# liron88/HM-16.2

Hardware: AMD Instinct MI355X
Metric: CTUs/sec (enc) at 4K main10; bit-exact CU partition vs HM (higher is better)
Workload: dtype int32+f64

## Files before the change

### hm-16.2_amd/csrc/hm355_core.h

```cpp
#pragma once
#include <stddef.h>
#include "hm355_types.h"

#ifdef HM355_HOSTSIM
#include <string.h>
#include <math.h>
#include <stdlib.h>
#define HM_DEV static
#define HM_FINL static inline
#define HM_FINL_M inline
#define HM_LAMBDA_INL
#define HM_NOINLINE __attribute__((noinline))
#define HM_CONST static const
#define HM_ASSUME_LDS(p) ((void)0)
#define HM_ASSUME_GLB(p) ((void)0)
#define HM_NT 1
static inline int hm_lane() { return 0; }
#define HM_SYNC() ((void)0)
static inline uint32_t hm_wave_sum(uint32_t v) { return v; }
static inline int hm_wave_sum_i(int v) { return v; }
static inline int hm_wave_max_i(int v) { return v; }
#define HM_UNI(x) (x)
#define HM_UCALL(x) (x)
#define hm_uni_ptr(p) (p)
// ... 217 lines not shown
struct TZ {
  const Pel *org; int orgStride, w, h;
  const Pel *ref; int refStride;
  uint32_t bestSad; int bestX, bestY, bestDist, bestRound, pointNr;
  int16_t l, r, t, b;
  int16_t subShift, pad_;
  int16_t lx[16], ly[16]; uint16_t lpd[16];
  int16_t wx0, wy0, ww, wh;
};
struct IrqFrame {
  TU t; int8_t phase, child, checkFull, checkSplit, zero; uint8_t bestTS[3];
  uint32_t absSum[3], bestCBF[3], singleBits, singleDist, subBits, subDist; double singleCost, subCost;
};

#define HM_TSTRIDE 33
#define HM_RQ_LDS 256
struct RqLds {
  int32_t lvl[HM_RQ_LDS];
  uint16_t pos[HM_RQ_LDS];
  uint16_t dec[HM_RQ_LDS];
  int16_t cur[HM_RQ_LDS];
  uint8_t ctxSig[HM_RQ_LDS];
  uint8_t code[HM_RQ_LDS];
  uint8_t cgCtxSet[64];
  uint8_t cgFlag[64];
};
struct RefLds {
  Pel refTop[2][132], refLeft[2][132];
  Pel refMain[200], refSide[200];
  Pel line[272];
};
#define HM_SLOT(d, ci) ((d) * CI_NUM + (ci) - ((d) == 4 ? 2 : 0))
#define HM_NUM_SLOTS (4 * CI_NUM + 3)
struct Team;
#if defined(HM355_PROFILE) && !defined(HM355_HOSTSIM)
#define HM_CTU_WAVES 11
#else
#define HM_CTU_WAVES 12
#endif
struct LdsTables {
  int8_t tmat[32 * HM_TSTRIDE];
  int8_t dst4[16];
  int32_t ebits[128];
};
#if defined(HM355_HOSTSIM)
static LdsTables g_lt;
#else
__shared__ LdsTables g_lt;
#endif
#define HM_LT() (&g_lt)
struct Shared {
  Cabac cur;
  int32_t bufA[32 * HM_TSTRIDE];
  union {
    int32_t bufB[32 * HM_TSTRIDE];
    RqLds rq;
    RefLds ref;
  } u;
  TuWalk walkOuter, walkInner;
  CuFrame cuf[4];
  double outCost; uint32_t outBits, outDist; double outRdCost;
  int32_t mpmZ;
  int32_t s8Winner, s8Reuse;
  InterMeta *im;
  uint32_t mcost; MvD mvPredictor; int32_t costScale;
  union {
// ... 1713 lines not shown
    }
    if (n == 4) {
      cabac_copy(&e->cur, &e->ws->slot[HM_SLOT(cuDepth, CI_CURR_BEST)]);
      { HM_PROF_BEGIN(e, PR_S4L); simt4_luma_pu(e, t, numModesForFullRD); HM_PROF_END(e, PR_S4L); }
      overallDistY += e->outDistY;
      if (pu != numPU - 1)
        par_copy_blk(e->fb.rec[0] + (e->ctuY * 64 + t.y) * ps + e->ctuX * 64 + t.x, ps, ws->reco + t.y * 64 + t.x, 64, n);
      continue;
    }
    int bestPUMode = 0; uint32_t bestPUDistY = 0; double bestPUCost = HM_MAX_DOUBLE;
    int firstPass = 0;
    if (n == 8 || n == 16) {
      cabac_copy(&e->cur, &e->ws->slot[HM_SLOT(cuDepth, CI_CURR_BEST)]);
      if (n == 8) { HM_PROF_BEGIN(e, PR_S8L); bestPUMode = HM_UCALL(simt8_luma_first_pass(e, t, numModesForFullRD)); HM_PROF_END(e, PR_S8L); }
      else { HM_PROF_BEGIN(e, PR_S16L); bestPUMode = HM_UCALL(simt16_luma_first_pass(e, t, numModesForFullRD)); HM_PROF_END(e, PR_S16L); }
      firstPass = numModesForFullRD;
      e->s8Reuse = 1;
    }
    for (int pass = firstPass; pass <= numModesForFullRD; pass++) {
      const int last = (pass == numModesForFullRD);
      const int orgMode = last ? bestPUMode : rdModeList[pass];
      par_set8(m->dirL + z, orgMode, puParts);
      cabac_copy(&e->cur, &e->ws->slot[HM_SLOT(cuDepth, CI_CURR_BEST)]);
      e->outCost = bestPUCost;
      if (last && n == 32 && numModesForFullRD > 0) { e->s8Reuse = 2; e->outDistY = bestPUDistY; e->outRdCost = bestPUCost; }
      recur_intra_coding_qt(e, t, !last);
      const uint32_t puDistY = e->outDistY; const double puCost = e->outRdCost;
      if (puCost < bestPUCost) {
        bestPUMode = orgMode; bestPUDistY = puDistY; bestPUCost = puCost;
        set_intra_result_qt(e, &t);
        HM_PAR_FOR(i, puParts) { ws->tmpTr[i] = m->tr[z + i]; for (int c = 0; c < 3; c++) { ws->tmpCbf[c][i] = m->cbf[c][z + i]; ws->tmpTs[c][i] = m->ts[c][z + i]; } }
        HM_SYNC();
        if (!last && n == 32) cabac_copy(&e->ws->slot[HM_SLOT(cuDepth, CI_QT_TRAFO_TEST)], &e->cur);
      }
    }
    overallDistY += bestPUDistY;
    HM_PAR_FOR(i, puParts) { m->tr[z + i] = ws->tmpTr[i]; for (int c = 0; c < 3; c++) { m->cbf[c][z + i] = ws->tmpCbf[c][i]; m->ts[c][z + i] = ws->tmpTs[c][i]; } m->dirL[z + i] = (uint8_t)bestPUMode; }
    HM_SYNC();
    if (pu != numPU - 1)
      par_copy_blk(e->fb.rec[0] + (e->ctuY * 64 + t.y) * ps + e->ctuX * 64 + t.x, ps, ws->reco + t.y * 64 + t.x, 64, n);
  }
  e->mpmZ = -1;
  if (numPU > 1) {
    uint8_t comb[3] = {0, 0, 0};
    for (int p = 0; p < 4; p++) for (int c = 0; c < 3; c++) comb[c] |= (m->cbf[c][cuZ + p * puParts] >> 1) & 1;
    HM_PAR_FOR(o, cuParts) for (int c = 0; c < 3; c++) m->cbf[c][cuZ + o] |= comb[c];
    HM_SYNC();
  }
  cabac_copy(&e->cur, &e->ws->slot[HM_SLOT(cuDepth, CI_CURR_BEST)]);
  return overallDistY;
}

HM_DEV inline uint32_t chroma_tu(Shared *e, const TU *t)
{
  CtuMeta *m = (&e->meta); const int z = t->cuZ + t->relZ;
  const int fullDepth = t->cuDepth + t->trDepth;
  int checkTS = (t->cW == 4) && (t->log2 == 2);
  if (checkTS) { int nb = 0; for (int s = 0; s < 4; s++) nb += m->ts[0][z + s]; checkTS = nb > 0; }
  const int zc = t->cuZ + t->cRelZ;
  if (t->cW == 4 && !checkTS) {
    cabac_copy(&e->ws->slot[HM_SLOT(fullDepth, CI_QT_TRAFO_ROOT)], &e->cur);
    HM_PROF_BEGIN(e, PR_S4CLEAF);
    const uint32_t d2 = HM_UCALL(simt4_chroma_leaf(e, *t));
    HM_PROF_END(e, PR_S4CLEAF);
    return d2;
  }
// ... 32 lines not shown
  const TU *root = &rootv;
  CtuMeta *m = (&e->meta);
  uint32_t dist = 0;
  tu_walk(e->walkOuter, root, 0,
    [&](const TU *t) {
      if (m->tr[t->cuZ + t->relZ] != t->trDepth) return 1;
      if (t->cW) dist += chroma_tu(e, t);
      return 0;
    },
    [&](const TU *t) {
      const int z = t->cuZ + t->relZ, q = t->parts >> 2;
      int any = 0;
      for (int c = 1; c < 3; c++) for (int s = 0; s < 4; s++) any |= ((m->cbf[c][z + s * q] >> (t->trDepth + 1)) & 1) << c;
      HM_PAR_FOR(o, t->parts) for (int c = 1; c < 3; c++) if ((any >> c) & 1) m->cbf[c][z + o] |= (uint8_t)(1 << t->trDepth);
      HM_SYNC();
    });
  return dist;
}
HM_DEV inline void set_intra_result_chroma_qt(Shared *e, const TU *root)
{
  const CtuMeta *m = (&e->meta);
  tu_walk(e->walkOuter, root, 0, [&](const TU *t) {
    if (!t->cW) return 0;
    if (m->tr[t->cuZ + t->relZ] != t->trDepth) return 1;
    const int n = t->cW, layer = 5 - t->log2;
    for (int c = 1; c < 3; c++) {
      const int po = HM_PLANE_OFF(c);
      par_copy32(e->cc + po + t->cOff, e->ws->qtCoef[layer] + po + t->cOff, n * n);
      par_copy_blk(e->ws->reco + po + t->cy * 32 + t->cx, 32, e->ws->qtRec[layer] + po + t->cy * 32 + t->cx, 32, n);
    }
    return 0;
  });
}
HM_DEV HM_NOINLINE uint32_t est_intra_pred_chroma_qt(Shared *e, int cuZ, int cuDepth)
{
  HM_ENTRY(e); cuZ = HM_UNI(cuZ); cuDepth = HM_UNI(cuDepth);
  CtuMeta *m = (&e->meta); WorkSpace *ws = e->ws; const int cuParts = 256 >> (2 * cuDepth);
  const TU t = tu_root(e, cuZ, cuDepth);
  if (cuDepth == 3) {
    const int split = m->tr[cuZ] != 0;
    int tsLuma = 0;
    if (split) for (int s = 0; s < 4; s++) tsLuma += m->ts[0][cuZ + s];
    if (!tsLuma) {
      cabac_copy(&e->cur, &e->ws->slot[HM_SLOT(cuDepth, CI_CURR_BEST)]);
      HM_PROF_BEGIN(e, PR_S4C);
      const uint32_t d = HM_UCALL(simt4_chroma_cu(e, split ? tu_child(&t, 0, 0) : t, cuZ));
      HM_PROF_END(e, PR_S4C);
      cabac_copy(&e->cur, &e->ws->slot[HM_SLOT(cuDepth, CI_CURR_BEST)]);
      return d;
    }
  }
  if (cuDepth == 2) {
    int split = 0;
    for (int i = 0; i < 16; i += 4) split |= m->tr[cuZ + i];
    if (!split) {
      cabac_copy(&e->cur, &e->ws->slot[HM_SLOT(cuDepth, CI_CURR_BEST)]);
      HM_PROF_BEGIN(e, PR_S8C);
      const uint32_t d = HM_UCALL(simt8_chroma_cu16(e, cuZ));
      HM_PROF_END(e, PR_S8C);
      cabac_copy(&e->cur, &e->ws->slot[HM_SLOT(cuDepth, CI_CURR_BEST)]);
      return d;
    }
  }
  int bestMode = 0; uint32_t bestDist = 0; double bestCost = HM_MAX_DOUBLE;
  int modeList[5];
  allowed_chroma_dirs(m->dirL[cuZ], modeList);
  for (int mi = 0; mi < 5; mi++) {
    cabac_copy(&e->cur, &e->ws->slot[HM_SLOT(cuDepth, CI_CURR_BEST)]);
    par_set8(m->dirC + cuZ, modeList[mi], cuParts);
    const uint32_t dist = HM_UCALL(recur_intra_chroma_coding_qt(e, t));
    cabac_copy(&e->cur, &e->ws->slot[HM_SLOT(cuDepth, CI_CURR_BEST)]);
    const uint32_t bits = HM_UCALL(intra_bits_qt(e, t, 0, 1));
    const double cost = calc_rd_cost(e, bits, dist);
    if (cost < bestCost) {
      bestCost = cost; bestDist = dist; bestMode = modeList[mi];
      set_intra_result_chroma_qt(e, &t);
      HM_PAR_FOR(i, cuParts) for (int c = 1; c < 3; c++) { ws->saveCbf[c][i] = m->cbf[c][cuZ + i]; ws->saveTs[c][i] = m->ts[c][cuZ + i]; }
      HM_SYNC();
    }
  }
  HM_PAR_FOR(i, cuParts) { for (int c = 1; c < 3; c++) { m->cbf[c][cuZ + i] = ws->saveCbf[c][i]; m->ts[c][cuZ + i] = ws->saveTs[c][i]; } m->dirC[cuZ + i] = (uint8_t)bestMode; }
  HM_SYNC();
  cabac_copy(&e->cur, &e->ws->slot[HM_SLOT(cuDepth, CI_CURR_BEST)]);
  return bestDist;
}

template <class C> HM_DEV inline void code_delta_qp(Shared *e, C *c, int dqp)
{
  const int off = 6 * (e->bitDepth - 8);
  dqp = (dqp + 78 + off + (off / 2)) % (52 + off) - 26 - (off / 2);
  const uint32_t a = (uint32_t)hm_abs(dqp), tu = a < 5 ? a : 5;
  enc_bin(e, c, C_DQP, tu ? 1 : 0);
  if (tu) { for (uint32_t k = tu; --k;) enc_bin(e, c, C_DQP + 1, 1); if (5 > tu) enc_bin(e, c, C_DQP + 1, 0); }
  if (a >= 5) {
    uint32_t sym = a - 5, count = 0, bins = 0; int nb = 0;
    while (sym >= (1u << count)) { bins = 2 * bins + 1; nb++; sym -= 1u << count; count++; }
    bins = 2 * bins; nb++;
    bins = (bins << count) | sym; nb += (int)count;
    enc_epv(c, bins, nb);
  }
  if (a > 0) enc_epv(c, dqp > 0 ? 0u : 1u, 1);
}
template <class C> HM_DEV inline void code_dqp_if_due(Shared *e, C *c)
{
  if (!e->fb.dqp) return;
  WorkSpace *ws = e->ws;
  if (!HM_UNI(ws->dq.flag)) return;
  code_delta_qp(e, c, HM_UNI(ws->dq.ctuQp) - HM_UNI(ws->dq.refQp));
// ... 83 lines not shown
  if (e->im) imeta_copy_range(&b->im, e->im, cuZ, parts);
  HM_PAR_FOR(i, parts * 16) b->coef[cuZ * 16 + i] = e->cc[cuZ * 16 + i];
  HM_PAR_FOR(i, parts * 4) { b->coef[4096 + cuZ * 4 + i] = e->cc[4096 + cuZ * 4 + i]; b->coef[5120 + cuZ * 4 + i] = e->cc[5120 + cuZ * 4 + i]; }
  const int r = hm_z2r(cuZ), x = (r & 15) * 4, y = (r >> 4) * 4, n = 64 >> cuDepth, l2 = 6 - cuDepth;
  HM_PAR_FOR(i, n * n) { const int yy = i >> l2, xx = i & (n - 1); b->reco[(y + yy) * 64 + x + xx] = e->ws->reco[(y + yy) * 64 + x + xx]; }
  HM_PAR_FOR(i, (n * n) >> 2) {
    const int yy = i >> (l2 - 1), xx = i & ((n >> 1) - 1), o = ((y >> 1) + yy) * 32 + (x >> 1) + xx;
    b->reco[4096 + o] = e->ws->reco[4096 + o]; b->reco[5120 + o] = e->ws->reco[5120 + o];
  }
  HM_SYNC();
  HM_PROF_END(e, PR_SAVE);
}
HM_DEV HM_NOINLINE void restore_best_from(Shared *e, const Best *b, int cuZ, int cuDepth)
{
  HM_ENTRY(e); cuZ = HM_UNI(cuZ); cuDepth = HM_UNI(cuDepth); b = hm_uni_ptr(b); HM_ASSUME_GLB(b);
  const int parts = 256 >> (2 * cuDepth);
  meta_copy_range((&e->meta), &b->m, cuZ, parts);
  if (e->im) imeta_copy_range(e->im, &b->im, cuZ, parts);
  HM_PAR_FOR(i, parts * 16) e->cc[cuZ * 16 + i] = b->coef[cuZ * 16 + i];
  HM_PAR_FOR(i, parts * 4) { e->cc[4096 + cuZ * 4 + i] = b->coef[4096 + cuZ * 4 + i]; e->cc[5120 + cuZ * 4 + i] = b->coef[5120 + cuZ * 4 + i]; }
  const int r = hm_z2r(cuZ), x = (r & 15) * 4, y = (r >> 4) * 4, n = 64 >> cuDepth, l2 = 6 - cuDepth;
  Pel *ry = e->fb.rec[0] + (e->ctuY * 64 + y) * e->stride[0] + e->ctuX * 64 + x;
  HM_PAR_FOR(i, n * n) { const int yy = i >> l2, xx = i & (n - 1); ry[yy * e->stride[0] + xx] = b->reco[(y + yy) * 64 + x + xx]; }
  Pel *ru = e->fb.rec[1] + (e->ctuY * 32 + (y >> 1)) * e->stride[1] + e->ctuX * 32 + (x >> 1);
  Pel *rv = e->fb.rec[2] + (e->ctuY * 32 + (y >> 1)) * e->stride[2] + e->ctuX * 32 + (x >> 1);
  HM_PAR_FOR(i, (n * n) >> 2) {
    const int yy = i >> (l2 - 1), xx = i & ((n >> 1) - 1), o = ((y >> 1) + yy) * 32 + (x >> 1) + xx;
    ru[yy * e->stride[1] + xx] = b->reco[4096 + o]; rv[yy * e->stride[2] + xx] = b->reco[5120 + o];
  }
  HM_SYNC();
}
HM_DEV inline void restore_best(Shared *e, int cuZ, int cuDepth) { restore_best_from(e, &e->ws->best[cuDepth], cuZ, cuDepth); }

HM_DEV HM_NOINLINE void check_rd_cost_intra(Shared *e, int cuZ, int cuDepth, int partSize)
{
  HM_ENTRY(e); cuZ = HM_UNI(cuZ); cuDepth = HM_UNI(cuDepth); partSize = HM_UNI(partSize);
  CtuMeta *m = (&e->meta); const int parts = 256 >> (2 * cuDepth);
#if defined(HM355_PROFILE) && !defined(HM355_HOSTSIM)
  const unsigned long long profCu0 = __builtin_readcyclecounter();
#endif
  init_est_data(e, cuZ, cuDepth);
  HM_PAR_FOR(i, parts) { m->part[cuZ + i] = (uint8_t)partSize; m->pred[cuZ + i] = MODE_INTRA; }
  HM_SYNC();
  HM_PROF_BEGIN(e, PR_LUMA);
  uint32_t d = HM_UCALL(est_intra_pred_qt(e, cuZ, cuDepth));
  HM_PROF_END(e, PR_LUMA);
  {
    const int r = hm_z2r(cuZ), x = (r & 15) * 4, y = (r >> 4) * 4, n = 64 >> cuDepth, ps = e->stride[0];
    par_copy_blk(e->fb.rec[0] + (e->ctuY * 64 + y) * ps + e->ctuX * 64 + x, ps, e->ws->reco + y * 64 + x, 64, n);
  }
  { HM_PROF_BEGIN(e, PR_CHROMA); d += HM_UCALL(est_intra_pred_chroma_qt(e, cuZ, cuDepth)); HM_PROF_END(e, PR_CHROMA); }
  reset_bits(&e->cur);
  { HM_PROF_BEGIN(e, PR_ENCCU); encode_cu_syntax(e, &e->cur, cuZ, cuDepth); HM_PROF_END(e, PR_ENCCU); }
  cabac_copy(&e->ws->slot[HM_SLOT(cuDepth, CI_TEMP_BEST)], &e->cur);
  e->outBits = num_bits(&e->cur); e->outDist = d;
  e->outCost = calc_rd_cost(e, e->outBits, e->outDist);
  check_dqp(e, cuZ, cuDepth);
#if defined(HM355_PROFILE) && !defined(HM355_HOSTSIM)
  { const int pid = partSize == SIZE_NxN ? PR_NXN : PR_D0 + cuDepth; e->prof[pid] += __builtin_readcyclecounter() - profCu0; e->profCnt[pid] += 1; }
#endif
}


#include "hm355_inter_cu.h"

template <class M> HM_FINL void cu_walk(Shared *e)
{
  CtuMeta *m = (&e->meta);
  CuFrame *fr = e->cuf; int sp = 0;
  fr[0].cuZ = 0; fr[0].phase = 0; fr[0].parentPart = SIZE_NONE;
  double retCost = 0; uint32_t retBits = 0, retDist = 0;
  M mode;
  while (sp >= 0) {
    CuFrame *f = &fr[sp]; const int cuDepth = sp, cuZ = f->cuZ;
    const int size = 64 >> cuDepth, parts = 256 >> (2 * cuDepth), q = parts >> 2;
    if (f->phase == 0) {
      const int r = hm_z2r(cuZ);
      const int lx = e->ctuX * 64 + (r & 15) * 4, ty = e->ctuY * 64 + (r >> 4) * 4;
      f->boundary = !((lx + size - 1 < e->width) && (ty + size - 1 < e->height));
      f->bestCost = HM_MAX_DOUBLE; f->bestBits = 0; f->bestDist = 0;
      if (mode.unsplit(e, f, cuZ, cuDepth)) { retCost = f->bestCost; retBits = f->bestBits; retDist = f->bestDist; sp--; continue; }
      init_est_data(e, cuZ, cuDepth);
      f->splitBits = 0; f->splitDist = 0; f->sub = 0; f->phase = 1;
    }
    if (f->phase == 1) {
      if (f->sub < 4) {
// ... 218 lines not shown
```

### hm-16.2_amd/csrc/hm355_simt.h

```cpp
#pragma once

template <int L2> struct SimtDim {
  enum { NC = 1 << (2 * L2), NCG = NC / 16, WCG = 1 << (L2 - 2), NSIG = L2 == 2 ? 9 : (L2 == 3 ? 21 : 27), NSET = NCG == 1 ? 1 : 4, NGRP = 2 * L2, NCGC = NCG == 1 ? 0 : 2,
         NLAST = L2 == 4 ? 4 : 3, LSH = L2 == 4 ? 1 : L2 - 2,
         X_SIG = 0, X_ONE = NSIG, X_ABS = X_ONE + 4 * NSET, X_LX = X_ABS + NSET, X_LY = X_LX + NLAST, X_CG = X_LY + NLAST, X_CBF = X_CG + NCGC,
         X_MODE = X_CBF + 1, X_TSKIP = X_MODE + 1, NCTX = X_TSKIP + (L2 == 2 ? 1 : 0),
         T_SIG = 0, T_ONE = 2 * NSIG, T_ABS = T_ONE + 8 * NSET, T_LASTX = T_ABS + 2 * NSET, T_LASTY = T_LASTX + NGRP, T_CG = T_LASTY + NGRP,
         T_CBF = T_CG + 2 * NCGC, T_N = T_CBF + 2 };
};
static_assert(SimtDim<2>::NCTX == 23 && SimtDim<2>::T_N == 38 && SimtDim<2>::X_LX == 14 && SimtDim<2>::X_LY == 17 && SimtDim<2>::X_CBF == 20 && SimtDim<2>::T_LASTX == 28 &&
              SimtDim<2>::T_LASTY == 32 && SimtDim<2>::T_CBF == 36 && SimtDim<2>::LSH == 0, "the 4x4 batch's numbering");
static_assert(SimtDim<3>::NCTX == 51 && SimtDim<3>::T_N == 100 && SimtDim<3>::X_ONE == 21 && SimtDim<3>::X_ABS == 37 && SimtDim<3>::X_LX == 41 && SimtDim<3>::X_LY == 44 &&
              SimtDim<3>::X_CG == 47 && SimtDim<3>::X_CBF == 49 && SimtDim<3>::T_ONE == 42 && SimtDim<3>::T_ABS == 74 && SimtDim<3>::T_LASTX == 82 && SimtDim<3>::T_LASTY == 88 &&
              SimtDim<3>::T_CG == 94 && SimtDim<3>::T_CBF == 98 && SimtDim<3>::LSH == 1 && SimtDim<3>::WCG == 2, "the 8x8 batch's numbering");
template <int L2> struct Simt;
template <int L2> struct SimtPrices {
  const int32_t *tab;
  HM_FINL_M int one(int i) const { return tab[SimtDim<L2>::T_ONE + i]; }
  HM_FINL_M int abs2(int i) const { return tab[SimtDim<L2>::T_ABS + i]; }
};

struct SimtPar {
  int chroma, bitDepth, qBits, quantCoef, tshift; double errScale, lambda; int64_t rdFactor;
  int dqShift, dqScale, dqMin, dqMax;
// ... 37 lines not shown
  if (j == D::X_CBF) return C_QT_CBF + cbfCodeCtx;
  if (j == D::X_MODE) return modeCtx;
  return C_TSKIP + (chroma ? 1 : 0);
}
template <int L2> HM_DEV inline void simt_setup(Shared *e, const Simt<L2> &S, const Cabac *cb, int jobs, int chroma, int cbfCtx, int cbfCodeCtx, int modeCtx)
{
  typedef SimtDim<L2> D;
  HM_PAR_FOR(i, D::T_N) {
    const int bin = i & 1;
    int v = 0;
    if (i < D::T_LASTX) {
      const int j = i >> 1, none = chroma && ((j < D::X_ONE && j >= 16) || (j >= D::X_ONE && j < D::X_ABS && j - D::X_ONE >= 8) || (j >= D::X_ABS && j - D::X_ABS >= 2));
      if (!none) v = HM_LT()->ebits[cb->s[simt_ctx_index<L2>(j, chroma, 0, 0)] ^ bin];
    } else if (i < D::T_CG) {
      const int g = (i - D::T_LASTX) % D::NGRP, x0 = i < D::T_LASTY ? D::X_LX : D::X_LY;
      for (int c = 0; c < g; c++) v += HM_LT()->ebits[cb->s[simt_ctx_index<L2>(x0 + (c >> D::LSH), chroma, 0, 0)] ^ 1];
      if (g < D::NGRP - 1) v += HM_LT()->ebits[cb->s[simt_ctx_index<L2>(x0 + (g >> D::LSH), chroma, 0, 0)] ^ 0];
      if (g > 3) v += 32768 * ((g - 2) >> 1);
    } else if (i < D::T_CBF) v = HM_LT()->ebits[cb->s[simt_ctx_index<L2>(D::X_CG + ((i - D::T_CG) >> 1), chroma, 0, 0)] ^ bin];
    else v = HM_LT()->ebits[cb->s[C_QT_CBF + cbfCtx] ^ bin];
    S.tab()[i] = v;
  }
  HM_PAR_FOR(i, 128) S.lps()[i] = HM_NEXT_LPS[i];
  HM_PAR_FOR(i, D::NCTX * S.JOBS) {
    const int j = i / S.JOBS, k = i - j * S.JOBS;
    if (k < jobs) S.ctx(j, k) = cb->s[simt_ctx_index<L2>(j, chroma, cbfCodeCtx, modeCtx)];
  }
  S.load_scans(e);
  HM_SYNC();
}
template <int L2> HM_FINL void simt_store_contexts(const Simt<L2> &S, int k, Cabac *cb, int cbfCodeCtx)
{
  HM_PAR_FOR(j, SimtDim<L2>::NCTX) cb->s[simt_ctx_index<L2>(j, 0, cbfCodeCtx, C_INTRA_LUMA)] = S.ctx(j, k);
}

template <int L2> HM_DEV inline void simt_bin(const Shared *e, const Simt<L2> &S, int k, uint32_t *frac, int c, int bin)
{
  const int st = S.ctx(c, k);
  *frac += (uint32_t)HM_LT()->ebits[st ^ bin];
  S.ctx(c, k) = (uint8_t)(bin == (st & 1) ? (st < 124 ? st + 2 : st) : S.lps()[st]);
}
template <int L2> HM_FINL int simt_cg_pattern(int cgBlkPos, int cgMask)
{
  const int W = SimtDim<L2>::WCG, cgx = cgBlkPos & (W - 1), cgy = cgBlkPos >> (L2 - 2);
  const int sigRight = cgx < W - 1 ? ((cgMask >> (cgBlkPos + 1)) & 1) : 0, sigLower = cgy < W - 1 ? ((cgMask >> (cgBlkPos + W)) & 1) : 0;
  return sigRight + (sigLower << 1);
}
template <int L2> HM_FINL void simt_last_xy(int blkPos, int scanType, int *px, int *py)
{
  const int y = blkPos >> L2, x = blkPos & ((1 << L2) - 1);
  *px = scanType == SCAN_VER ? y : x; *py = scanType == SCAN_VER ? x : y;
}

template <int L2> HM_DEV inline int simt_rdoq(const Simt<L2> &S, const SimtPar &p, int k, int scanType)
{
  typedef SimtDim<L2> D;
  const int32_t *tab = S.tab(); const SimtPrices<L2> prices = { tab };
  const int qBits = p.qBits, half = 1 << (qBits - 1);
  const double lambda = p.lambda, errScale = p.errScale;
  const int firstCtx = first_sig_ctx(1 << L2, scanType, p.chroma), lumaSets = p.chroma ? 0 : 2;
  double blockUncoded = 0, baseCost = 0;
  int last = -1, cgLast = -1, ctxSet = 0;
  int cgMask = 0; uint32_t cgSets = 0;
  LevelChain ch;
  for (int cg = D::NCG - 1; cg >= 0; cg--) {
    const int cgBlkPos = S.cg_pos(scanType, cg), cgBit = 1 << cgBlkPos, pattern = simt_cg_pattern<L2>(cgBlkPos, cgMask);
// ... 253 lines not shown
```

### hm-16.2_amd/csrc/hm355_simt4.h

```cpp
#pragma once

#define HM_SL 22
struct Simt4A {
  double cost[16][HM_SL];
  double outCost[HM_SL];
  uint32_t outDist[HM_SL], outBits[HM_SL];
  int32_t tab[SimtDim<2>::T_N];
  uint8_t ctx[SimtDim<2>::NCTX][HM_SL];
  uint8_t outCbf[HM_SL];
  uint8_t lps[128];
};
struct Simt4B {
  int32_t cs[16][HM_SL];
  int32_t dc[16][HM_SL];
  uint8_t scan[3][16];
  uint8_t sigIdx[3][16];
};
static_assert(sizeof(Simt4A) <= sizeof(((Shared *)0)->bufA), "Simt4A overlays bufA");
static_assert(offsetof(RefLds, refMain) + sizeof(Simt4B) <= sizeof(((Shared *)0)->u), "Simt4B overlays the tail of the LDS union");
static_assert(offsetof(RefLds, refMain) % 8 == 0, "alignment of the overlay");
HM_DEV constexpr int s4_scan(int type, int i)
{
  constexpr uint8_t t[3][16] = { {0, 4, 1, 8, 5, 2, 12, 9, 6, 3, 13, 10, 7, 14, 11, 15}, {0, 1, 2, 3, 4, 5, 6, 7, 8, 9, 10, 11, 12, 13, 14, 15},
                                 {0, 4, 8, 12, 1, 5, 9, 13, 2, 6, 10, 14, 3, 7, 11, 15} };
// ... 216 lines not shown
  const int lumaDir = m->dirL[cuZ];
  allowed_chroma_dirs(lumaDir, modeList);
  const Simt4 S(e); Simt4A *A = S.A;
  simt_setup(e, S, &e->cur, 10, 1, 5 + t->trDepth, 5, C_CHROMA_PRED);
  const SimtPar p = simt_params<2>(e, 1);
  const uint32_t baseFrac = (uint32_t)(e->cur.frac & 32767);
  const int dcVal[2] = { ref_dc_val(e, 0, 4), ref_dc_val(e, 1, 4) };
  HM_LVA(int32_t, rec, 16); HM_LVA(int32_t, lv, 16);
  HM_WAVE_FOR(k) {
    if (k < 10) {
      const int c = k & 1, mi = k >> 1, ps = e->stride[1 + c];
      const int dirC = chroma_mode_at(modeList, mi), mode = dirC == DM_CHROMA_IDX ? lumaDir : dirC, scanType = intra_scan_type(mode);
      const Pel *org = e->fb.org[1 + c] + (size_t)py * ps + px;
      int cbf;
      const uint32_t sse = s4_eval(e, S, p, k, c, org, ps, mode, 0, scanType, c ? dcVal[1] : dcVal[0], HM_LVAK(rec, k), HM_LVAK(lv, k), &cbf);
      A->outDist[k] = (uint32_t)(e->fb.chromaWeight * (double)sse);
      A->outCbf[k] = (uint8_t)cbf;
    }
  }
  HM_SYNC();
  HM_WAVE_FOR(k) {
    if (k < 10 && !(k & 1)) {
      const int mi = k >> 1;
      const int dirC = chroma_mode_at(modeList, mi), mode = dirC == DM_CHROMA_IDX ? lumaDir : dirC, scanType = intra_scan_type(mode);
      uint32_t frac = baseFrac;
      simt_bin(e, S, k, &frac, SimtDim<2>::X_MODE, dirC != DM_CHROMA_IDX);
      if (dirC != DM_CHROMA_IDX) frac += 2u * 32768u;
      const int cbfU = A->outCbf[k], cbfV = A->outCbf[k + 1];
      simt_bin(e, S, k, &frac, SimtDim<2>::X_CBF, cbfU);
      simt_bin(e, S, k, &frac, SimtDim<2>::X_CBF, cbfV);
      if (cbfU) s4_code_coeff(e, S, k, k, 1, scanType, 0, &frac);
      if (cbfV) s4_code_coeff(e, S, k, k + 1, 1, scanType, 0, &frac);
      const uint32_t bits = frac >> 15, dist = A->outDist[k] + A->outDist[k + 1];
      A->outBits[k] = dist;
      A->outCost[k] = calc_rd_cost(e, bits, dist);
    }
  }
  HM_SYNC();
  double bestCost = HM_MAX_DOUBLE; int best = 0;
  for (int mi = 0; mi < 5; mi++) { const double c = A->outCost[2 * mi]; if (c < bestCost) { bestCost = c; best = mi; } }
  best = HM_UNI(best);
  const uint32_t bestDist = A->outBits[2 * best];
  const int cbfU = A->outCbf[2 * best], cbfV = A->outCbf[2 * best + 1];
  HM_WAVE_FOR(k) {
    if ((k >> 1) == best && k < 10) {
      const int po = HM_PLANE_OFF(1 + (k & 1));
      TCoeff *coef = e->cc + po + t->cOff; Pel *ro = ws->reco + po + t->cy * 32 + t->cx;
#pragma unroll
      for (int i = 0; i < 16; i++) { coef[i] = HM_LVAK(lv, k)[i]; ro[(i >> 2) * 32 + (i & 3)] = (Pel)HM_LVAK(rec, k)[i]; }
    }
  }
  {
    const int vU = t->trDepth ? 3 * cbfU : cbfU, vV = t->trDepth ? 3 * cbfV : cbfV, bm = chroma_mode_at(modeList, best);
    HM_PAR_FOR(i, 4) { m->cbf[1][cuZ + i] = (uint8_t)vU; m->cbf[2][cuZ + i] = (uint8_t)vV; m->ts[1][cuZ + i] = 0; m->ts[2][cuZ + i] = 0; m->dirC[cuZ + i] = (uint8_t)bm; }
  }
  HM_SYNC();
  return bestDist;
}

HM_DEV HM_NOINLINE void simt4_luma_leaf(Shared *e, TU tv)
{
  HM_ENTRY(e); tv = hm_uni_struct(tv);
  const TU *t = &tv; CtuMeta *m = (&e->meta); WorkSpace *ws = e->ws;
  const int z = t->cuZ + t->relZ, ps = e->stride[0], r = hm_z2r(z), mode = m->dirL[z];
  init_adi_pattern(e, 0, e->ctuX * 64 + t->x, e->ctuY * 64 + t->y, 4, e->ctuX * 16 + (r & 15), e->ctuY * 16 + (r >> 4), 1, 0);
  {
    CabacR cr; cabr_load(e, cr, &e->cur);
    cr.frac &= 32767;
    enc_intra_header(e, &cr, t, 1, 0);
    cabr_store(cr, &e->cur);
  }
  const Simt4 S(e); Simt4A *A = S.A;
  simt_setup(e, S, &e->cur, 1, 0, 0, 0, C_INTRA_LUMA);
  const SimtPar p = simt_params<2>(e, 0);
  const Pel *org = e->fb.org[0] + (e->ctuY * 64 + t->y) * ps + e->ctuX * 64 + t->x;
  const int dcVal = ref_dc_val(e, 0, 4);
  const int scanType = intra_scan_type(mode);
  const uint32_t frac0 = (uint32_t)e->cur.frac;
  HM_WAVE_FOR(k) {
    if (k == 0) {
      int32_t rec[16], lv[16]; int cbf;
      const uint32_t dist = s4_eval(e, S, p, 0, 0, org, ps, mode, 0, scanType, dcVal, rec, lv, &cbf);
      uint32_t frac = frac0;
      simt_bin(e, S, 0, &frac, SimtDim<2>::X_CBF, cbf);
      if (cbf) s4_code_coeff(e, S, 0, 0, 0, scanType, 0, &frac);
      A->outDist[0] = dist; A->outBits[0] = frac; A->outCbf[0] = (uint8_t)cbf;
      TCoeff *coef = ws->qtCoef[3] + z * 16; Pel *rq = ws->qtRec[3] + t->y * 64 + t->x;
      Pel *recPic = e->fb.rec[0] + (e->ctuY * 64 + t->y) * ps + e->ctuX * 64 + t->x;
// ... 49 lines not shown
```

### hm-16.2_amd/csrc/hm355_simt8.h

```cpp
#pragma once

#define HM_S8 11
struct Simt8A {
  int32_t tile[2][64];
  int32_t tab[SimtDim<3>::T_N];
  double outCost[HM_S8];
  uint32_t outDist[HM_S8], outFrac[HM_S8];
  int16_t cs[64][HM_S8];
  uint8_t ctx[SimtDim<3>::NCTX][HM_S8];
  uint8_t outCbf[HM_S8], best;
  uint8_t lps[128];
};
struct Simt8B {
  int32_t dc[64][HM_S8];
  uint8_t scan[3][64];
  uint8_t scanCG[3][4];
};
static_assert(sizeof(Simt8A) <= sizeof(((Shared *)0)->bufA), "Simt8A overlays bufA");
static_assert(offsetof(RefLds, refMain) + sizeof(Simt8B) <= sizeof(((Shared *)0)->u), "Simt8B overlays the tail of the LDS union");
template <> struct Simt<3> {
  enum { JOBS = HM_S8, KEEPS_COST = 0 };
  Simt8A *A; Simt8B *B;
  HM_FINL_M explicit Simt(Shared *e) : A((Simt8A *)e->bufA), B((Simt8B *)((char *)&e->u + offsetof(RefLds, refMain))) {}
  HM_FINL_M int32_t *tab() const { return A->tab; }
// ... 142 lines not shown
  const int x4 = e->ctuX * 16 + (r & 15), y4 = e->ctuY * 16 + (r >> 4), px = e->ctuX * 32 + t.cx, py = e->ctuY * 32 + t.cy;
  simt_chroma_ref_lines(e, px, py, 8, x4, y4);
  int modeList[5];
  const int lumaDir = m->dirL[cuZ];
  allowed_chroma_dirs(lumaDir, modeList);
  const Simt8 S(e); Simt8A *A = S.A;
  simt_setup(e, S, &e->cur, 10, 1, 5, 5, C_CHROMA_PRED);
  const SimtPar p = simt_params<3>(e, 1);
  const uint32_t baseFrac = (uint32_t)(e->cur.frac & 32767);
  const int dcVal[2] = { ref_dc_val(e, 0, 8), ref_dc_val(e, 1, 8) };
  const int shiftSse = (bitDepth - 8) << 1;
  for (int job = 0; job < 10; job++) {
    const int c = job & 1, dirC = modeList[job >> 1], mode = dirC == DM_CHROMA_IDX ? lumaDir : dirC, ps = e->stride[1 + c];
    s8_residual_fwd(S, e->fb.org[1 + c] + (size_t)py * ps + px, ps, bitDepth, SCAN_DIAG, job,
                    [&](int x, int y) HM_LAMBDA_INL { return s8_pred_sample_chroma(e, c, mode, x, y, dcVal[c]); });
  }
  HM_WAVE_FOR(k) { if (k < 10) A->outCbf[k] = (uint8_t)(simt_rdoq(S, p, k, SCAN_DIAG) > 0); }
  HM_SYNC();
  for (int pass = 0; pass < 12; pass++) {
    int job = pass;
    if (pass == 10) {
      HM_WAVE_FOR(k) {
        if (k < 10 && !(k & 1)) {
          const int dirC = modeList[k >> 1];
          uint32_t frac = baseFrac;
          simt_bin(e, S, k, &frac, SimtDim<3>::X_MODE, dirC != DM_CHROMA_IDX);
          if (dirC != DM_CHROMA_IDX) frac += 2u * 32768u;
          const int cbfU = A->outCbf[k], cbfV = A->outCbf[k + 1];
          simt_bin(e, S, k, &frac, SimtDim<3>::X_CBF, cbfU);
          simt_bin(e, S, k, &frac, SimtDim<3>::X_CBF, cbfV);
          if (cbfU) simt_code_coeff(e, S, k, k, 1, SCAN_DIAG, &frac);
          if (cbfV) simt_code_coeff(e, S, k, k + 1, 1, SCAN_DIAG, &frac);
          const uint32_t dist = A->outDist[k] + A->outDist[k + 1];
          A->outCost[k] = calc_rd_cost(e, frac >> 15, dist);
        }
      }
      HM_SYNC();
      double bestCost = HM_MAX_DOUBLE; int best = 0;
      for (int mi = 0; mi < 5; mi++) { const double v = A->outCost[2 * mi]; if (v < bestCost) { bestCost = v; best = mi; } }
      best = HM_UNI(best);
      if (hm_lane() == 0) A->best = (uint8_t)best;
      HM_SYNC();
    }
    const int best = pass >= 10 ? A->best : 0;
    if (pass >= 10) job = 2 * best + (pass - 10);
    const int c = job & 1, dirC = modeList[job >> 1], mode = dirC == DM_CHROMA_IDX ? lumaDir : dirC, ps = e->stride[1 + c], cbf = A->outCbf[job];
    const Pel *org = e->fb.org[1 + c] + (size_t)py * ps + px;
    const int po = HM_PLANE_OFF(1 + c);
    s8_dequant_inv1(S, p, SCAN_DIAG, job, cbf, pass >= 10 ? e->cc + po + t.cOff : (TCoeff *)0);
    uint32_t sse = 0;
    s8_inv2_recon(S, bitDepth, cbf, [&](int x, int y) HM_LAMBDA_INL { return s8_pred_sample_chroma(e, c, mode, x, y, dcVal[c]); },
                  [&](int x, int y, int rr) HM_LAMBDA_INL {
                    const int d = org[y * ps + x] - rr; sse += (uint32_t)((d * d) >> shiftSse);
                    if (pass >= 10) ws->reco[po + (t.cy + y) * 32 + t.cx + x] = (Pel)rr;
                  });
    const uint32_t dsum = hm_wave_sum(sse);
    if (pass < 10 && hm_lane() == 0) A->outDist[job] = (uint32_t)(e->fb.chromaWeight * (double)dsum);
    HM_SYNC();
  }
  const int best = A->best, cbfU = A->outCbf[2 * best], cbfV = A->outCbf[2 * best + 1];
  const uint32_t bestDist = A->outDist[2 * best] + A->outDist[2 * best + 1];
  const int bm = modeList[best];
  HM_PAR_FOR(i, 16) { m->cbf[1][cuZ + i] = (uint8_t)cbfU; m->cbf[2][cuZ + i] = (uint8_t)cbfV; m->ts[1][cuZ + i] = 0; m->ts[2][cuZ + i] = 0; m->dirC[cuZ + i] = (uint8_t)bm; }
  HM_SYNC();
  return bestDist;
}
```

### hm-16.2_amd/csrc/hm355_types.h

```cpp
#pragma once
#include <stdint.h>

typedef int16_t Pel;
typedef int32_t TCoeff;

enum {
  C_SPLIT = 0, C_PART = 3, C_INTRA_LUMA = 7, C_CHROMA_PRED = 8, C_SUBDIV = 10, C_QT_CBF = 13, C_SIG_CG = 23,
  C_SIG = 27, C_LASTX = 71, C_LASTY = 101, C_ONE = 131, C_ABS = 155, C_TSKIP = 161,
   C_SKIP = 163, C_MRG_FLAG = 166, C_MRG_IDX = 167, C_PRED_MODE = 168, C_INTER_DIR = 169, C_MVD = 174, C_REF = 176,
  C_ROOT_CBF = 178, C_MVP_IDX = 179,  C_DQP = 180, HM_NUM_CTX = 183
};
struct Cabac {
  uint8_t s[184];
  uint64_t frac;
};
enum { CI_CURR_BEST = 0, CI_NEXT_BEST, CI_TEMP_BEST, CI_QT_TRAFO_TEST, CI_QT_TRAFO_ROOT, CI_NUM };

struct CtuMeta {
  uint8_t depth[256], part[256], pred[256], dirL[256], dirC[256], tr[256], cbf[3][256], ts[3][256];
};
struct CtuStat { double cost; uint32_t bits, dist; };
struct MvD { int16_t x, y; };
struct InterMeta {
  uint8_t skip[256], mrg[256], mrgIdx[256], interDir[256];
  MvD mv[2][256], mvd[2][256];
  int8_t refIdx[2][256], mvpIdx[2][256], mvpNum[2][256];
};
#define HM_REF_MARGIN 80
struct RefPicDev {
  const Pel *plane[3];
  int32_t stride[3];
  int32_t poc, isLongTerm;
  const uint8_t *predMode;
  const MvD *mv[2]; const int8_t *refIdx[2];
  int32_t refPoc[2][16], refLT[2][16];
};
struct InterPic {
  int32_t sliceType, poc, numRefIdx[2];
  RefPicDev ref[2][16];
  int32_t colFromL0, colRefIdx, tmvp, mvdL1Zero, maxMergeCand, checkLDC, cabacInitType;
  uint32_t lambdaMotionSAD, lambdaMotionSSE;
  MvD integerMv2Nx2N[2][16];
  int32_t list1ToList0[16];
};

#define HM_PLANE_OFF(c) ((c) == 0 ? 0 : ((c) == 1 ? 4096 : 5120))
#define HM_PLANE_STRIDE(c) ((c) == 0 ? 64 : 32)
#define HM_TEAM 9
#define HM_TEAM_I 5
#define HM_COEF_CTU 6144

struct Best {
  CtuMeta m;
  InterMeta im;
  TCoeff coef[HM_COEF_CTU];
  Pel reco[HM_COEF_CTU];
};

struct WorkSpace {
  Best best[4];
  Pel pred[HM_COEF_CTU], resi[HM_COEF_CTU], reco[HM_COEF_CTU];
  Pel qtRec[4][HM_COEF_CTU];
  TCoeff qtCoef[4][HM_COEF_CTU];
  MvD intMv[2][16];
  Pel tsPred[3][16], tsRec[3][16]; TCoeff tsCoef[3][16];
  double costCoeff[1024];
  Cabac slot[4 * CI_NUM + 3];
  Pel tmpPred[HM_COEF_CTU];
  Pel resiBest[HM_COEF_CTU];
  Pel mcTmp[72 * 64];
  Pel mcBlk[64 * 64];
  Pel yuvPred[2][HM_COEF_CTU];
  Pel orgBi[64 * 64];
  struct PuSearch {
    MvD mvTemp[2][16], mvPred[2][16], mvPredBi[2][16], cand[2][16][2];
    int8_t mvpIdx[2][16], mvpIdxBi[2][16], mvpNum[2][16];
    uint32_t costTempL0[16], bitsTempL0[16];
  } ps;
  struct { MvD mv[5][2]; int32_t ref[5][2]; uint8_t dir[5]; int32_t num; } mrg2N;
  uint8_t tmpTr[256], tmpCbf[3][256], tmpTs[3][256], saveCbf[3][256], saveTs[3][256];
  struct { int32_t ctuQp, refQp, flag, pad; } dq;
  TCoeff teamCoef[HM_COEF_CTU];
  InterMeta teamIm;
  MvD teamTok[3][2][16];
};

struct QpTab { int32_t qpPer[2], qpRem[2]; double errScale[2][4]; int64_t rdFactor[2]; };
struct CtuDqp {
  int8_t qp, refQp, lastQp;
  uint8_t flagOut;
  int16_t firstZ, pad;
};
struct CtuRc {
  double lambda, sqrtLambda, lambdaC;
  int64_t rdFactor[2];
  uint32_t lambdaMotionSAD, lambdaMotionSSE;
};
struct CtuRcOut { int32_t bits, qp; };
struct DqpPic {
  int32_t flagIn, sliceQp;
// ... 50 lines not shown
```

Baseline: 25860.

## Reuse luma and chroma search CABAC states instead of re-encoding CU syntax

In intra 2Nx2N checks without inter or dQP, the CU's final CABAC context state and fractional bit count are built by merging the saved states from the winning luma pass and the winning chroma pass. This replaces a full encode_cu_syntax recount. A partial chroma-only re-encode is used when the split root has both chroma CBFs set. The SIMT chroma kernels now export the winner's contexts and frac so the merge is possible. A host-side diagnostic checks the merge is bit-exact against a full recount. The risk is subtle bit mismatches if the context ownership table or the frac arithmetic is wrong.

```diff
diff --git a/hm-16.2_amd/csrc/hm355_core.h b/hm-16.2_amd/csrc/hm355_core.h
--- a/hm-16.2_amd/csrc/hm355_core.h
+++ b/hm-16.2_amd/csrc/hm355_core.h
@@ -273,6 +273,8 @@
 };
 #define HM_SLOT(d, ci) ((d) * CI_NUM + (ci) - ((d) == 4 ? 2 : 0))
 #define HM_NUM_SLOTS (4 * CI_NUM + 3)
+#define HM_SLOT_CU_LUMA HM_NUM_SLOTS
+#define HM_SLOT_CU_CHROMA (HM_NUM_SLOTS + 1)
 struct Team;
 #if defined(HM355_PROFILE) && !defined(HM355_HOSTSIM)
 #define HM_CTU_WAVES 11
@@ -2052,6 +2054,7 @@
         HM_PAR_FOR(i, puParts) { ws->tmpTr[i] = m->tr[z + i]; for (int c = 0; c < 3; c++) { ws->tmpCbf[c][i] = m->cbf[c][z + i]; ws->tmpTs[c][i] = m->ts[c][z + i]; } }
         HM_SYNC();
         if (!last && n == 32) cabac_copy(&e->ws->slot[HM_SLOT(cuDepth, CI_QT_TRAFO_TEST)], &e->cur);
+        if (!nxn && !e->im) cabac_copy(&e->ws->slot[HM_SLOT_CU_LUMA], &e->cur);
       }
     }
     overallDistY += bestPUDistY;
@@ -2150,8 +2153,15 @@
     return 0;
   });
 }
+#if defined(HM355_CHECK_CU_BITS)
+static int g_cub_chroma_path;
+#define HM_CUB_CHROMA_PATH(v) (g_cub_chroma_path = (v))
+#else
+#define HM_CUB_CHROMA_PATH(v) ((void)0)
+#endif
 HM_DEV HM_NOINLINE uint32_t est_intra_pred_chroma_qt(Shared *e, int cuZ, int cuDepth)
 {
+  HM_CUB_CHROMA_PATH(0);
   HM_ENTRY(e); cuZ = HM_UNI(cuZ); cuDepth = HM_UNI(cuDepth);
   CtuMeta *m = (&e->meta); WorkSpace *ws = e->ws; const int cuParts = 256 >> (2 * cuDepth);
   const TU t = tu_root(e, cuZ, cuDepth);
@@ -2162,8 +2172,10 @@
     if (!tsLuma) {
       cabac_copy(&e->cur, &e->ws->slot[HM_SLOT(cuDepth, CI_CURR_BEST)]);
       HM_PROF_BEGIN(e, PR_S4C);
+      HM_CUB_CHROMA_PATH(1);
       const uint32_t d = HM_UCALL(simt4_chroma_cu(e, split ? tu_child(&t, 0, 0) : t, cuZ));
       HM_PROF_END(e, PR_S4C);
+      cabac_copy(&e->ws->slot[HM_SLOT_CU_CHROMA], &e->cur);
       cabac_copy(&e->cur, &e->ws->slot[HM_SLOT(cuDepth, CI_CURR_BEST)]);
       return d;
     }
@@ -2174,8 +2186,10 @@
     if (!split) {
       cabac_copy(&e->cur, &e->ws->slot[HM_SLOT(cuDepth, CI_CURR_BEST)]);
       HM_PROF_BEGIN(e, PR_S8C);
+      HM_CUB_CHROMA_PATH(2);
       const uint32_t d = HM_UCALL(simt8_chroma_cu16(e, cuZ));
       HM_PROF_END(e, PR_S8C);
+      cabac_copy(&e->ws->slot[HM_SLOT_CU_CHROMA], &e->cur);
       cabac_copy(&e->cur, &e->ws->slot[HM_SLOT(cuDepth, CI_CURR_BEST)]);
       return d;
     }
@@ -2192,6 +2206,7 @@
     const double cost = calc_rd_cost(e, bits, dist);
     if (cost < bestCost) {
       bestCost = cost; bestDist = dist; bestMode = modeList[mi];
+      cabac_copy(&e->ws->slot[HM_SLOT_CU_CHROMA], &e->cur);
       set_intra_result_chroma_qt(e, &t);
       HM_PAR_FOR(i, cuParts) for (int c = 1; c < 3; c++) { ws->saveCbf[c][i] = m->cbf[c][cuZ + i]; ws->saveTs[c][i] = m->ts[c][cuZ + i]; }
       HM_SYNC();
@@ -2341,6 +2356,90 @@
 }
 HM_DEV inline void restore_best(Shared *e, int cuZ, int cuDepth) { restore_best_from(e, &e->ws->best[cuDepth], cuZ, cuDepth); }
 
+enum { CUB_RECOUNT = 0, CUB_MERGE, CUB_CHROMA_RECOUNT };
+HM_DEV inline int cu_bits_class(const Shared *e, int cuZ, int cuDepth, int partSize)
+{
+  if (partSize != SIZE_2Nx2N || e->im || e->fb.dqp) return CUB_RECOUNT;
+  const CtuMeta *m = (&e->meta);
+  if (cuDepth < 3 && m->tr[cuZ] != 0 && (m->cbf[1][cuZ] & 1) && (m->cbf[2][cuZ] & 1)) return CUB_CHROMA_RECOUNT;
+  return CUB_MERGE;
+}
+HM_DEV inline int hm_is_chroma_ctx(int i)
+{
+#define HM_CHROMA_CTX_IN(a, b) || (i >= (a) && i < (b))
+  return 0 HM_CHROMA_CTX_TABLE(HM_CHROMA_CTX_IN);
+#undef HM_CHROMA_CTX_IN
+}
+HM_DEV HM_NOINLINE void encode_cu_chroma_syntax(Shared *e, int cuZ, int cuDepth)
+{
+  HM_ENTRY(e); cuZ = HM_UNI(cuZ); cuDepth = HM_UNI(cuDepth);
+  const CtuMeta *m = (&e->meta); Cabac *c = &e->cur;
+  code_intra_dir_chroma(e, c, cuZ);
+  const TU root = tu_root(e, cuZ, cuDepth);
+  tu_walk(e->walkOuter, &root, 1, [&](const TU *t) {
+    const int subdiv = m->tr[t->cuZ + t->relZ] > t->trDepth;
+    code_chroma_cbfs(e, c, t, subdiv);
+    if (subdiv) return 1;
+    for (int comp = 1; comp < 3; comp++) code_tu_coeff(e, c, t, comp, e->cc, 1);
+    return 0;
+  });
+}
+HM_DEV inline void cu_bits_from_passes(Shared *e, int cuZ, int cuDepth, int how)
+{
+  const Cabac *L = &e->ws->slot[HM_SLOT_CU_LUMA], *C = &e->ws->slot[HM_SLOT_CU_CHROMA];
+  if (how == CUB_CHROMA_RECOUNT) {
+    cabac_copy(&e->cur, L);
+    encode_cu_chroma_syntax(e, cuZ, cuDepth);
+    return;
+  }
+  const uint64_t *lp = (const uint64_t *)L, *cp = (const uint64_t *)C; uint64_t *dp = (uint64_t *)&e->cur;
+  HM_PAR_FOR(i, (int)(sizeof(Cabac) / 8)) {
+    if (i == (int)(offsetof(Cabac, frac) / 8)) dp[i] = lp[i] + cp[i] - (dp[i] & 32767);
+    else {
+      uint64_t mask = 0;
+      for (int b = 0; b < 8; b++) if (hm_is_chroma_ctx(8 * i + b)) mask |= 0xffull << (8 * b);
+      dp[i] = (lp[i] & ~mask) | (cp[i] & mask);
+    }
+  }
+  HM_SYNC();
+}
+#if defined(HM355_CHECK_CU_BITS)
+#ifndef HM355_HOSTSIM
+#error "HM355_CHECK_CU_BITS is a diagnostic of the host twin"
+#endif
+#include <stdio.h>
+#include <stdlib.h>
+#include <unistd.h>
+static unsigned long long g_cub_n[3], g_cub_bad;
+static void cu_bits_report(void)
+{
+  fprintf(stderr, "CU_BITS merged %llu chroma_recount %llu recount %llu mismatch %llu\n", g_cub_n[CUB_MERGE], g_cub_n[CUB_CHROMA_RECOUNT], g_cub_n[CUB_RECOUNT], g_cub_bad);
+  fflush(stderr);
+  if (g_cub_bad) _exit(3);
+}
+static inline void cu_bits_check(Shared *e, int cuZ, int cuDepth, int partSize, int how)
+{
+  static int registered = 0;
+  if (!registered) { registered = 1; atexit(cu_bits_report); }
+  if (partSize != SIZE_2Nx2N || e->im) return;
+  g_cub_n[how]++;
+  if (how == CUB_RECOUNT) return;
+  const Cabac got = e->cur;
+  cabac_copy(&e->cur, &e->ws->slot[HM_SLOT(cuDepth, CI_CURR_BEST)]);
+  reset_bits(&e->cur);
+  encode_cu_syntax(e, &e->cur, cuZ, cuDepth);
+  int firstBad = -1;
+  for (int i = HM_NUM_CTX - 1; i >= 0; i--) if (got.s[i] != e->cur.s[i]) firstBad = i;
+  if (firstBad < 0 && got.frac == e->cur.frac) return;
+  g_cub_bad++;
+  const CtuMeta *m = (&e->meta);
+  static const char *const chromaPath[3] = { "wave-uniform", "simt4_chroma_cu", "simt8_chroma_cu16" };
+  const char *closing = m->tr[cuZ] ? "split root" : (cuDepth >= 2 ? "winner's lane (s8Reuse 1)" : "parked first pass (s8Reuse 2)");
+  fprintf(stderr, "CU_BITS mismatch: frame CTU %d cuZ %d depth %d class %d, luma closing: %s, chroma: %s; frac %llu, recount %llu; first context that differs %d\n",
+          e->ctuAddr, cuZ, cuDepth, how, closing, chromaPath[g_cub_chroma_path], (unsigned long long)got.frac, (unsigned long long)e->cur.frac, firstBad);
+}
+#endif
+
 HM_DEV HM_NOINLINE void check_rd_cost_intra(Shared *e, int cuZ, int cuDepth, int partSize)
 {
   HM_ENTRY(e); cuZ = HM_UNI(cuZ); cuDepth = HM_UNI(cuDepth); partSize = HM_UNI(partSize);
@@ -2359,8 +2458,14 @@
     par_copy_blk(e->fb.rec[0] + (e->ctuY * 64 + y) * ps + e->ctuX * 64 + x, ps, e->ws->reco + y * 64 + x, 64, n);
   }
   { HM_PROF_BEGIN(e, PR_CHROMA); d += HM_UCALL(est_intra_pred_chroma_qt(e, cuZ, cuDepth)); HM_PROF_END(e, PR_CHROMA); }
-  reset_bits(&e->cur);
-  { HM_PROF_BEGIN(e, PR_ENCCU); encode_cu_syntax(e, &e->cur, cuZ, cuDepth); HM_PROF_END(e, PR_ENCCU); }
+  HM_PROF_BEGIN(e, PR_ENCCU);
+  const int how = cu_bits_class(e, cuZ, cuDepth, partSize);
+  if (how == CUB_RECOUNT) { reset_bits(&e->cur); encode_cu_syntax(e, &e->cur, cuZ, cuDepth); }
+  else cu_bits_from_passes(e, cuZ, cuDepth, how);
+  HM_PROF_END(e, PR_ENCCU);
+#if defined(HM355_CHECK_CU_BITS)
+  cu_bits_check(e, cuZ, cuDepth, partSize, how);
+#endif
   cabac_copy(&e->ws->slot[HM_SLOT(cuDepth, CI_TEMP_BEST)], &e->cur);
   e->outBits = num_bits(&e->cur); e->outDist = d;
   e->outCost = calc_rd_cost(e, e->outBits, e->outDist);
diff --git a/hm-16.2_amd/csrc/hm355_simt.h b/hm-16.2_amd/csrc/hm355_simt.h
--- a/hm-16.2_amd/csrc/hm355_simt.h
+++ b/hm-16.2_amd/csrc/hm355_simt.h
@@ -93,6 +93,15 @@
 template <int L2> HM_FINL void simt_store_contexts(const Simt<L2> &S, int k, Cabac *cb, int cbfCodeCtx)
 {
   HM_PAR_FOR(j, SimtDim<L2>::NCTX) cb->s[simt_ctx_index<L2>(j, 0, cbfCodeCtx, C_INTRA_LUMA)] = S.ctx(j, k);
+}
+template <int L2> HM_FINL void simt_store_chroma_mode(const Simt<L2> &S, int k, Cabac *cb, uint32_t frac)
+{
+  typedef SimtDim<L2> D;
+  HM_PAR_FOR(j, D::NCTX) {
+    const int none = (j < D::X_ONE && j >= 16) || (j >= D::X_ONE && j < D::X_ABS && j - D::X_ONE >= 8) || (j >= D::X_ABS && j < D::X_LX && j - D::X_ABS >= 2);
+    if (!none) cb->s[simt_ctx_index<L2>(j, 1, 5, C_CHROMA_PRED)] = S.ctx(j, k);
+  }
+  cb->frac = (uint64_t)frac;
 }
 
 template <int L2> HM_DEV inline void simt_bin(const Shared *e, const Simt<L2> &S, int k, uint32_t *frac, int c, int bin)
diff --git a/hm-16.2_amd/csrc/hm355_simt4.h b/hm-16.2_amd/csrc/hm355_simt4.h
--- a/hm-16.2_amd/csrc/hm355_simt4.h
+++ b/hm-16.2_amd/csrc/hm355_simt4.h
@@ -272,7 +272,7 @@
       if (cbfU) s4_code_coeff(e, S, k, k, 1, scanType, 0, &frac);
       if (cbfV) s4_code_coeff(e, S, k, k + 1, 1, scanType, 0, &frac);
       const uint32_t bits = frac >> 15, dist = A->outDist[k] + A->outDist[k + 1];
-      A->outBits[k] = dist;
+      A->outBits[k] = dist; A->outBits[k + 1] = frac;
       A->outCost[k] = calc_rd_cost(e, bits, dist);
     }
   }
@@ -294,6 +294,7 @@
     const int vU = t->trDepth ? 3 * cbfU : cbfU, vV = t->trDepth ? 3 * cbfV : cbfV, bm = chroma_mode_at(modeList, best);
     HM_PAR_FOR(i, 4) { m->cbf[1][cuZ + i] = (uint8_t)vU; m->cbf[2][cuZ + i] = (uint8_t)vV; m->ts[1][cuZ + i] = 0; m->ts[2][cuZ + i] = 0; m->dirC[cuZ + i] = (uint8_t)bm; }
   }
+  simt_store_chroma_mode(S, 2 * best, &e->cur, A->outBits[2 * best + 1]);
   HM_SYNC();
   return bestDist;
 }
diff --git a/hm-16.2_amd/csrc/hm355_simt8.h b/hm-16.2_amd/csrc/hm355_simt8.h
--- a/hm-16.2_amd/csrc/hm355_simt8.h
+++ b/hm-16.2_amd/csrc/hm355_simt8.h
@@ -198,6 +198,7 @@
           if (cbfU) simt_code_coeff(e, S, k, k, 1, SCAN_DIAG, &frac);
           if (cbfV) simt_code_coeff(e, S, k, k + 1, 1, SCAN_DIAG, &frac);
           const uint32_t dist = A->outDist[k] + A->outDist[k + 1];
+          A->outFrac[k] = frac;
           A->outCost[k] = calc_rd_cost(e, frac >> 15, dist);
         }
       }
@@ -228,6 +229,7 @@
   const uint32_t bestDist = A->outDist[2 * best] + A->outDist[2 * best + 1];
   const int bm = modeList[best];
   HM_PAR_FOR(i, 16) { m->cbf[1][cuZ + i] = (uint8_t)cbfU; m->cbf[2][cuZ + i] = (uint8_t)cbfV; m->ts[1][cuZ + i] = 0; m->ts[2][cuZ + i] = 0; m->dirC[cuZ + i] = (uint8_t)bm; }
+  simt_store_chroma_mode(S, 2 * best, &e->cur, A->outFrac[2 * best]);
   HM_SYNC();
   return bestDist;
 }
diff --git a/hm-16.2_amd/csrc/hm355_types.h b/hm-16.2_amd/csrc/hm355_types.h
--- a/hm-16.2_amd/csrc/hm355_types.h
+++ b/hm-16.2_amd/csrc/hm355_types.h
@@ -14,6 +14,16 @@
   uint8_t s[184];
   uint64_t frac;
 };
+#define HM_CHROMA_CTX_TABLE(X) \
+  X(C_CHROMA_PRED, C_SUBDIV)          \
+  X(C_QT_CBF + 5, C_SIG_CG)           \
+  X(C_SIG_CG + 2, C_SIG)              \
+  X(C_SIG + 28, C_LASTX)              \
+  X(C_LASTX + 15, C_LASTY)            \
+  X(C_LASTY + 15, C_ONE)              \
+  X(C_ONE + 16, C_ABS)                \
+  X(C_ABS + 4, C_TSKIP)               \
+  X(C_TSKIP + 1, C_SKIP)
 enum { CI_CURR_BEST = 0, CI_NEXT_BEST, CI_TEMP_BEST, CI_QT_TRAFO_TEST, CI_QT_TRAFO_ROOT, CI_NUM };
 
 struct CtuMeta {
@@ -65,7 +75,7 @@
   MvD intMv[2][16];
   Pel tsPred[3][16], tsRec[3][16]; TCoeff tsCoef[3][16];
   double costCoeff[1024];
-  Cabac slot[4 * CI_NUM + 3];
+  Cabac slot[4 * CI_NUM + 3 + 2];
   Pel tmpPred[HM_COEF_CTU];
   Pel resiBest[HM_COEF_CTU];
   Pel mcTmp[72 * 64];
```

New measurement: 26570 (median of 6 runs). +2.7%, better.
